# sczhou/CodeFormer

Hardware: AMD Instinct MI355X
Metric: aligned 512x512 faces/sec (whole node) at w=0.5 (higher is better)
Workload: dtype f32; 1 GPU; BASELINE config 2 (IEEE fp32 arithmetic): 16 faces/GPU, w=0.5, adain, seed-0 random-init weights; global_batch=16, parallelism=single GPU, precision=fp32

## Files before the change

### codeformer_amd/csrc/cf_gemm_split.hip

```cpp
#include <cstdlib>
#include <type_traits>

#include "cf_common.h"

namespace {

typedef _Float16 gs_f16x8 __attribute__((ext_vector_type(8)));

struct GsArgs {
  const float* a;
  const float* w;
  const float* bias;
  const float* res;
  float* out;
  int M, N, K;
  int epilogue;
  float acc_scale;
  float* ws;
  unsigned* counters;
  int nsplit;
  const float* a_alt;
  int n_alt;
};
__device__ __forceinline__ const float* gs_rows(const GsArgs& g, int n0) { return (g.a_alt && n0 >= g.n_alt) ? g.a_alt : g.a; }

constexpr int GS_GROUP = 4;

__global__ __launch_bounds__(256) void gemm_split_kernel(const GsArgs g) {
  __shared__ float s_flag;
  const int tid = threadIdx.x, lane = tid & 63, wave = tid >> 6;
  const int wm = wave >> 1, wn = wave & 1;
  const int half = lane >> 5, l31 = lane & 31;
  int bid = blockIdx.x;
  const int split = bid % g.nsplit;
  const int tile = bid / g.nsplit;
  const int ntn = g.N >> 6;
  const int nt = tile % ntn, mt = tile / ntn;
  const int m0 = mt * 64 + wm * 32, n0 = nt * 64 + wn * 32;
  const int V = g.K >> 7;
  const int nv = V / g.nsplit;
  const int c0 = split * nv;

  const float* const arow = gs_rows(g, n0) + (size_t)(m0 + l31) * g.K + half * 8 + (size_t)c0 * 128;
  const size_t kstride = (size_t)(g.N >> 5) * 512;
  const float* const wl = g.w + (size_t)(n0 >> 5) * 512 + lane * 4 + (size_t)c0 * 8 * kstride;

  f32x4 ra[2][GS_GROUP][2], rb[2][GS_GROUP][2];
  auto fetch = [&](int grp, auto buf) __attribute__((always_inline)) {
    constexpr int BUF = decltype(buf)::value;
#pragma unroll
    for (int s = 0; s < GS_GROUP; ++s) {
      const int ks = grp * GS_GROUP + s;
      ra[BUF][s][0] = *reinterpret_cast<const f32x4*>(arow + ks * 16);
      ra[BUF][s][1] = *reinterpret_cast<const f32x4*>(arow + ks * 16 + 4);
      rb[BUF][s][0] = *reinterpret_cast<const f32x4*>(wl + (size_t)ks * kstride);
      rb[BUF][s][1] = *reinterpret_cast<const f32x4*>(wl + (size_t)ks * kstride + 256);
    }
  };
  f32x16 acc, tot;
#pragma unroll
  for (int r = 0; r < 16; ++r) acc[r] = tot[r] = 0.f;
  auto compute = [&](auto buf) __attribute__((always_inline)) {
    constexpr int BUF = decltype(buf)::value;
#pragma unroll
    for (int s = 0; s < GS_GROUP; ++s) {
      f32x4 ah, al;
#pragma unroll
      for (int e = 0; e < 4; ++e) {
        const f32x4 v = ra[BUF][s][e >> 1];
        float hh, ll;
        cf_split_pair(v[(e & 1) * 2], v[(e & 1) * 2 + 1], hh, ll);
        ah[e] = hh;
        al[e] = ll;
      }
      acc = __builtin_amdgcn_mfma_f32_32x32x16_f16(__builtin_bit_cast(gs_f16x8, al), __builtin_bit_cast(gs_f16x8, rb[BUF][s][0]), acc, 0, 0, 0);
      acc = __builtin_amdgcn_mfma_f32_32x32x16_f16(__builtin_bit_cast(gs_f16x8, ah), __builtin_bit_cast(gs_f16x8, rb[BUF][s][1]), acc, 0, 0, 0);
      acc = __builtin_amdgcn_mfma_f32_32x32x16_f16(__builtin_bit_cast(gs_f16x8, ah), __builtin_bit_cast(gs_f16x8, rb[BUF][s][0]), acc, 0, 0, 0);
    }
  };

  using B0 = std::integral_constant<int, 0>;
  using B1 = std::integral_constant<int, 1>;
  const int ngroups = nv * 2;
  fetch(0, B0{});
  for (int c = 0; c < nv; ++c) {
    fetch(2 * c + 1, B1{});
    __builtin_amdgcn_sched_barrier(0);
    compute(B0{});
    if (2 * c + 2 < ngroups) fetch(2 * c + 2, B0{});
    __builtin_amdgcn_sched_barrier(0);
    compute(B1{});
    if (g.nsplit == 1) {
#pragma unroll
      for (int r = 0; r < 16; ++r) tot[r] += acc[r];
    } else {
      f32x4 v[4];
#pragma unroll
      for (int i = 0; i < 4; ++i) v[i] = f32x4{acc[4 * i], acc[4 * i + 1], acc[4 * i + 2], acc[4 * i + 3]};
      cf_splitk_park(v, g.ws, tile, c0 + c, V, 256);
    }
#pragma unroll
    for (int r = 0; r < 16; ++r) acc[r] = 0.f;
  }
  if (g.nsplit > 1) {
    f32x4 v[4];
    if (!cf_splitk_finish(v, g.ws, g.counters, tile, V, g.nsplit, 256, &s_flag)) return;
#pragma unroll
    for (int i = 0; i < 4; ++i)
#pragma unroll
      for (int e = 0; e < 4; ++e) tot[4 * i + e] = v[i][e];
  }

  const int n = n0 + l31;
  const float bias = g.bias ? g.bias[n] : 0.f;
#pragma unroll
  for (int r = 0; r < 16; ++r) {
    const size_t o = (size_t)(m0 + cf_acc_row(r, lane)) * g.N + n;
    float v = tot[r] * g.acc_scale + bias;
    if (g.epilogue == CF_EPI_GELU) v = 0.5f * v * (1.0f + erff(v * 0.70710678118654752440f));
    if (g.epilogue == CF_EPI_RESIDUAL) v += g.res[o];
    g.out[o] = v;
  }
}

template <int NI>
__global__ __launch_bounds__(256) void gemm_split_tile_kernel(const GsArgs g) {
  constexpr int BN = 64 * NI;
  __shared__ __attribute__((aligned(16))) float As[2][2][128][16];
  const int tid = threadIdx.x, lane = tid & 63, wave = __builtin_amdgcn_readfirstlane(tid >> 6);
  const int wm = wave >> 1, wn = wave & 1;
  const int half = lane >> 5, l31 = lane & 31;
  const int ntn = g.N / BN;
  const int nt = blockIdx.x % ntn, mt = blockIdx.x / ntn;
  const int m0 = mt * 128, n0 = nt * BN + wn * (32 * NI);
  const int nst = g.K >> 5;

  const float* const asrc = gs_rows(g, n0) + (size_t)(m0 + (tid >> 3)) * g.K + (tid & 7) * 4;
  f32x4 rg[4][4];
  auto load_stage = [&](int st, auto buf) __attribute__((always_inline)) {
    constexpr int BUF = decltype(buf)::value;
#pragma unroll
    for (int j = 0; j < 4; ++j) rg[BUF][j] = *reinterpret_cast<const f32x4*>(asrc + (size_t)(32 * j) * g.K + st * 32);
  };
  typedef float gs_f32x2 __attribute__((ext_vector_type(2)));
  auto store_stage = [&](int lbuf, auto buf) __attribute__((always_inline)) {
    constexpr int BUF = decltype(buf)::value;
    const int q = tid & 7, ks = q >> 2, hf = (q >> 1) & 1, sub = q & 1;
#pragma unroll
    for (int j = 0; j < 4; ++j) {
      const int row = (tid >> 3) + 32 * j;
      const int swz = (row >> 2) & 3;
      float h0, l0, h1, l1;
      cf_split_pair(rg[BUF][j][0], rg[BUF][j][1], h0, l0);
      cf_split_pair(rg[BUF][j][2], rg[BUF][j][3], h1, l1);
      float* base = &As[lbuf][ks][row][0];
      *reinterpret_cast<gs_f32x2*>(base + ((hf ^ swz) << 2) + sub * 2) = gs_f32x2{h0, h1};
      *reinterpret_cast<gs_f32x2*>(base + (((2 + hf) ^ swz) << 2) + sub * 2) = gs_f32x2{l0, l1};
    }
  };
  const size_t kstride = (size_t)(g.N >> 5) * 512;
  const float* const wl = g.w + (size_t)(n0 >> 5) * 512 + lane * 4;
  f32x4 rb[4][2][NI][2];
  auto load_B = [&](int st, auto buf) __attribute__((always_inline)) {
    constexpr int BUF = decltype(buf)::value;
#pragma unroll
    for (int s = 0; s < 2; ++s)
#pragma unroll
      for (int ni = 0; ni < NI; ++ni) {
        const float* p = wl + (size_t)(st * 2 + s) * kstride + ni * 512;
        rb[BUF][s][ni][0] = *reinterpret_cast<const f32x4*>(p);
        rb[BUF][s][ni][1] = *reinterpret_cast<const f32x4*>(p + 256);
      }
  };
  f32x16 acc[2][NI], tot[2][NI];
#pragma unroll
  for (int mi = 0; mi < 2; ++mi)
#pragma unroll
    for (int ni = 0; ni < NI; ++ni)
#pragma unroll
      for (int r = 0; r < 16; ++r) acc[mi][ni][r] = tot[mi][ni][r] = 0.f;
  auto compute = [&](int lbuf, auto buf) __attribute__((always_inline)) {
    constexpr int BUF = decltype(buf)::value;
#pragma unroll
    for (int s = 0; s < 2; ++s) {
      f32x4 ah[2], al[2];
#pragma unroll
      for (int mi = 0; mi < 2; ++mi) {
        const int row = wm * 64 + mi * 32 + l31;
        const int swz = (row >> 2) & 3;
        ah[mi] = *reinterpret_cast<const f32x4*>(&As[lbuf][s][row][(half ^ swz) << 2]);
        al[mi] = *reinterpret_cast<const f32x4*>(&As[lbuf][s][row][((2 + half) ^ swz) << 2]);
      }
#pragma unroll
      for (int mi = 0; mi < 2; ++mi)
#pragma unroll
        for (int ni = 0; ni < NI; ++ni) {
          acc[mi][ni] = __builtin_amdgcn_mfma_f32_32x32x16_f16(__builtin_bit_cast(gs_f16x8, al[mi]), __builtin_bit_cast(gs_f16x8, rb[BUF][s][ni][0]), acc[mi][ni], 0, 0, 0);
          acc[mi][ni] = __builtin_amdgcn_mfma_f32_32x32x16_f16(__builtin_bit_cast(gs_f16x8, ah[mi]), __builtin_bit_cast(gs_f16x8, rb[BUF][s][ni][1]), acc[mi][ni], 0, 0, 0);
          acc[mi][ni] = __builtin_amdgcn_mfma_f32_32x32x16_f16(__builtin_bit_cast(gs_f16x8, ah[mi]), __builtin_bit_cast(gs_f16x8, rb[BUF][s][ni][0]), acc[mi][ni], 0, 0, 0);
        }
    }
  };
  using R0 = std::integral_constant<int, 0>;
  using R1 = std::integral_constant<int, 1>;
  using R2 = std::integral_constant<int, 2>;
  using R3 = std::integral_constant<int, 3>;
  auto stage = [&](int st, auto cur, auto nxt, auto far, auto do_load, auto do_store) __attribute__((always_inline)) {
    if constexpr (decltype(do_load)::value) {
      load_stage(st + 3, far);
      load_B(st + 3, far);
    }
    __builtin_amdgcn_sched_barrier(0);
    compute(st & 1, cur);
    if ((st & 3) == 3) {
#pragma unroll
      for (int mi = 0; mi < 2; ++mi)
#pragma unroll
        for (int ni = 0; ni < NI; ++ni)
#pragma unroll
          for (int r = 0; r < 16; ++r) {
            tot[mi][ni][r] += acc[mi][ni][r];
            acc[mi][ni][r] = 0.f;
          }
    }
    if constexpr (decltype(do_store)::value) store_stage((st + 1) & 1, nxt);
    __syncthreads();
  };
  constexpr std::true_type Y{};
  constexpr std::false_type NO{};
  load_stage(0, R0{});
  load_B(0, R0{});
  load_stage(1, R1{});
  load_B(1, R1{});
  load_stage(2, R2{});
  load_B(2, R2{});
  store_stage(0, R0{});
  __syncthreads();
  int st = 0;
  for (; st + 4 < nst; st += 4) {
    stage(st, R0{}, R1{}, R3{}, Y, Y);
    stage(st + 1, R1{}, R2{}, R0{}, Y, Y);
    stage(st + 2, R2{}, R3{}, R1{}, Y, Y);
    stage(st + 3, R3{}, R0{}, R2{}, Y, Y);
  }
  stage(st, R0{}, R1{}, R3{}, Y, Y);
  stage(st + 1, R1{}, R2{}, R0{}, NO, Y);
  stage(st + 2, R2{}, R3{}, R1{}, NO, Y);
  stage(st + 3, R3{}, R0{}, R2{}, NO, NO);

#pragma unroll
  for (int ni = 0; ni < NI; ++ni) {
    const int n = n0 + ni * 32 + l31;
    const float bias = g.bias ? g.bias[n] : 0.f;
#pragma unroll
    for (int mi = 0; mi < 2; ++mi)
#pragma unroll
      for (int r = 0; r < 16; ++r) {
        const size_t o = (size_t)(m0 + wm * 64 + mi * 32 + cf_acc_row(r, lane)) * g.N + n;
        float v = tot[mi][ni][r] * g.acc_scale + bias;
        if (g.epilogue == CF_EPI_GELU) v = 0.5f * v * (1.0f + erff(v * 0.70710678118654752440f));
        if (g.epilogue == CF_EPI_RESIDUAL) v += g.res[o];
        g.out[o] = v;
      }
  }
}

constexpr int GS_CHUNK_MAXV = 8;
template <int MI, int NI>
__global__ __launch_bounds__(256, MI * NI == 1 ? 1 : 2) void gemm_split_chunk_kernel(const GsArgs g) {
  extern __shared__ __attribute__((aligned(16))) float gs_part[];
  constexpr int HS = MI * NI == 1 ? 8 : 4;
  const int tid = threadIdx.x, lane = tid & 63, wave = __builtin_amdgcn_readfirstlane(tid >> 6);
  const int half = lane >> 5, l31 = lane & 31;
  const int ntn = g.N / (32 * NI);
  const int nt = blockIdx.x % ntn, mt = blockIdx.x / ntn;
  const int m0 = mt * (32 * MI), n0 = nt * (32 * NI);
  const int V = g.K >> 7;
  const float* const arow = gs_rows(g, n0) + (size_t)(m0 + l31) * g.K + half * 8;
  const size_t kstride = (size_t)(g.N >> 5) * 512;
  const float* const wl = g.w + (size_t)(n0 >> 5) * 512 + lane * 4;
  for (int c = wave; c < V; c += 4) {
    f32x16 acc[MI][NI];
#pragma unroll
    for (int mi = 0; mi < MI; ++mi)
#pragma unroll
      for (int ni = 0; ni < NI; ++ni)
#pragma unroll
        for (int r = 0; r < 16; ++r) acc[mi][ni][r] = 0.f;
#pragma unroll
    for (int h = 0; h < 8 / HS; ++h) {
      f32x4 ra[HS][MI][2], rb[HS][NI][2];
#pragma unroll
      for (int s = 0; s < HS; ++s) {
        const int ks = c * 8 + h * HS + s;
#pragma unroll
        for (int mi = 0; mi < MI; ++mi) {
          ra[s][mi][0] = *reinterpret_cast<const f32x4*>(arow + (size_t)(32 * mi) * g.K + ks * 16);
          ra[s][mi][1] = *reinterpret_cast<const f32x4*>(arow + (size_t)(32 * mi) * g.K + ks * 16 + 4);
        }
#pragma unroll
        for (int ni = 0; ni < NI; ++ni) {
          rb[s][ni][0] = *reinterpret_cast<const f32x4*>(wl + (size_t)ks * kstride + ni * 512);
          rb[s][ni][1] = *reinterpret_cast<const f32x4*>(wl + (size_t)ks * kstride + ni * 512 + 256);
        }
      }
      __builtin_amdgcn_sched_barrier(0);
#pragma unroll
      for (int s = 0; s < HS; ++s) {
        f32x4 ah[MI], al[MI];
#pragma unroll
        for (int mi = 0; mi < MI; ++mi)
#pragma unroll
          for (int e = 0; e < 4; ++e) {
            const f32x4 v = ra[s][mi][e >> 1];
            float hh, ll;
            cf_split_pair(v[(e & 1) * 2], v[(e & 1) * 2 + 1], hh, ll);
            ah[mi][e] = hh;
            al[mi][e] = ll;
          }
#pragma unroll
        for (int mi = 0; mi < MI; ++mi)
#pragma unroll
          for (int ni = 0; ni < NI; ++ni) {
            acc[mi][ni] = __builtin_amdgcn_mfma_f32_32x32x16_f16(__builtin_bit_cast(gs_f16x8, al[mi]), __builtin_bit_cast(gs_f16x8, rb[s][ni][0]), acc[mi][ni], 0, 0, 0);
            acc[mi][ni] = __builtin_amdgcn_mfma_f32_32x32x16_f16(__builtin_bit_cast(gs_f16x8, ah[mi]), __builtin_bit_cast(gs_f16x8, rb[s][ni][1]), acc[mi][ni], 0, 0, 0);
            acc[mi][ni] = __builtin_amdgcn_mfma_f32_32x32x16_f16(__builtin_bit_cast(gs_f16x8, ah[mi]), __builtin_bit_cast(gs_f16x8, rb[s][ni][0]), acc[mi][ni], 0, 0, 0);
          }
      }
    }
#pragma unroll
    for (int mi = 0; mi < MI; ++mi)
#pragma unroll
      for (int ni = 0; ni < NI; ++ni)
#pragma unroll
        for (int r = 0; r < 16; ++r) gs_part[(((c * MI + mi) * NI + ni) * 16 + r) * 64 + lane] = acc[mi][ni][r];
  }
  __syncthreads();
#pragma unroll
  for (int ni = 0; ni < NI; ++ni) {
    const int n = n0 + ni * 32 + l31;
    const float bias = g.bias ? g.bias[n] : 0.f;
#pragma unroll
    for (int mi = 0; mi < MI; ++mi)
#pragma unroll
      for (int j = 0; j < 4; ++j) {
        const int r = wave + 4 * j;
        float tot = 0.f;
        for (int c = 0; c < V; ++c) tot += gs_part[(((c * MI + mi) * NI + ni) * 16 + r) * 64 + lane];
        const size_t o = (size_t)(m0 + mi * 32 + cf_acc_row(r, lane)) * g.N + n;
        float v = tot * g.acc_scale + bias;
        if (g.epilogue == CF_EPI_GELU) v = 0.5f * v * (1.0f + erff(v * 0.70710678118654752440f));
        if (g.epilogue == CF_EPI_RESIDUAL) v += g.res[o];
        g.out[o] = v;
      }
  }
}

__global__ __launch_bounds__(256) void gemm_f32_tile_kernel(const GsArgs g) {
  __shared__ __attribute__((aligned(16))) float As[2][2][128][16];
  const int tid = threadIdx.x, lane = tid & 63, wave = __builtin_amdgcn_readfirstlane(tid >> 6);
  const int wm = wave >> 1, wn = wave & 1;
  const int half = lane >> 5, l31 = lane & 31;
  const int ntn = g.N / 64;
  const int nt = blockIdx.x % ntn, mt = blockIdx.x / ntn;
  const int m0 = mt * 128, n0 = nt * 64 + wn * 32;
  const int nst = g.K >> 5;

  const float* const asrc = gs_rows(g, n0) + (size_t)(m0 + (tid >> 3)) * g.K + (tid & 7) * 4;
  f32x4 rg[4][4];
  auto load_stage = [&](int st, auto buf) __attribute__((always_inline)) {
    constexpr int BUF = decltype(buf)::value;
#pragma unroll
    for (int j = 0; j < 4; ++j) rg[BUF][j] = *reinterpret_cast<const f32x4*>(asrc + (size_t)(32 * j) * g.K + st * 32);
  };
  auto store_stage = [&](int lbuf, auto buf) __attribute__((always_inline)) {
    constexpr int BUF = decltype(buf)::value;
    const int q = tid & 7, ks = q >> 2, ch = q & 3;
#pragma unroll
    for (int j = 0; j < 4; ++j) {
      const int row = (tid >> 3) + 32 * j;
      *reinterpret_cast<f32x4*>(&As[lbuf][ks][row][(ch ^ ((row >> 2) & 3)) << 2]) = rg[BUF][j];
    }
  };
  const float* const wl = g.w + (size_t)(n0 + l31) * 16 + half * 4;
  const size_t kstride = (size_t)g.N * 16;
  f32x4 rb[4][2][2];
  auto load_B = [&](int st, auto buf) __attribute__((always_inline)) {
    constexpr int BUF = decltype(buf)::value;
#pragma unroll
    for (int s = 0; s < 2; ++s) {
      const float* p = wl + (size_t)(st * 2 + s) * kstride;
      rb[BUF][s][0] = *reinterpret_cast<const f32x4*>(p);
      rb[BUF][s][1] = *reinterpret_cast<const f32x4*>(p + 8);
    }
  };
  f32x16 acc[2], tot[2];
#pragma unroll
  for (int mi = 0; mi < 2; ++mi)
#pragma unroll
    for (int r = 0; r < 16; ++r) acc[mi][r] = tot[mi][r] = 0.f;
  auto compute = [&](int lbuf, auto buf) __attribute__((always_inline)) {
    constexpr int BUF = decltype(buf)::value;
#pragma unroll
    for (int s = 0; s < 2; ++s) {
      f32x4 a0[2], a1[2];
#pragma unroll
      for (int mi = 0; mi < 2; ++mi) {
        const int row = wm * 64 + mi * 32 + l31;
        const int swz = (row >> 2) & 3;
        a0[mi] = *reinterpret_cast<const f32x4*>(&As[lbuf][s][row][(half ^ swz) << 2]);
        a1[mi] = *reinterpret_cast<const f32x4*>(&As[lbuf][s][row][((2 + half) ^ swz) << 2]);
      }
#pragma unroll
      for (int j = 0; j < 4; ++j)
#pragma unroll
        for (int mi = 0; mi < 2; ++mi) acc[mi] = __builtin_amdgcn_mfma_f32_32x32x2f32(a0[mi][j], rb[BUF][s][0][j], acc[mi], 0, 0, 0);
#pragma unroll
      for (int j = 0; j < 4; ++j)
#pragma unroll
        for (int mi = 0; mi < 2; ++mi) acc[mi] = __builtin_amdgcn_mfma_f32_32x32x2f32(a1[mi][j], rb[BUF][s][1][j], acc[mi], 0, 0, 0);
    }
  };
  using R0 = std::integral_constant<int, 0>;
  using R1 = std::integral_constant<int, 1>;
  using R2 = std::integral_constant<int, 2>;
  using R3 = std::integral_constant<int, 3>;
  auto stage = [&](int st, auto cur, auto nxt, auto far, auto do_load, auto do_store) __attribute__((always_inline)) {
    if constexpr (decltype(do_load)::value) {
      load_stage(st + 3, far);
      load_B(st + 3, far);
    }
    __builtin_amdgcn_sched_barrier(0);
    compute(st & 1, cur);
    if ((st & 3) == 3) {
#pragma unroll
      for (int mi = 0; mi < 2; ++mi) {
        tot[mi] += acc[mi];
#pragma unroll
        for (int r = 0; r < 16; ++r) acc[mi][r] = 0.f;
      }
    }
    if constexpr (decltype(do_store)::value) store_stage((st + 1) & 1, nxt);
    __syncthreads();
  };
  constexpr std::true_type Y{};
  constexpr std::false_type NO{};
  load_stage(0, R0{});
  load_B(0, R0{});
  load_stage(1, R1{});
  load_B(1, R1{});
  load_stage(2, R2{});
  load_B(2, R2{});
  store_stage(0, R0{});
  __syncthreads();
  int st = 0;
  for (; st + 4 < nst; st += 4) {
    stage(st, R0{}, R1{}, R3{}, Y, Y);
    stage(st + 1, R1{}, R2{}, R0{}, Y, Y);
    stage(st + 2, R2{}, R3{}, R1{}, Y, Y);
    stage(st + 3, R3{}, R0{}, R2{}, Y, Y);
  }
  stage(st, R0{}, R1{}, R3{}, Y, Y);
  stage(st + 1, R1{}, R2{}, R0{}, NO, Y);
  stage(st + 2, R2{}, R3{}, R1{}, NO, Y);
  stage(st + 3, R3{}, R0{}, R2{}, NO, NO);

  const int n = n0 + l31;
  const float bias = g.bias ? g.bias[n] : 0.f;
#pragma unroll
  for (int mi = 0; mi < 2; ++mi)
#pragma unroll
    for (int r = 0; r < 16; ++r) {
      const size_t o = (size_t)(m0 + wm * 64 + mi * 32 + cf_acc_row(r, lane)) * g.N + n;
      float v = tot[mi][r] + bias;
      if (g.epilogue == CF_EPI_GELU) v = 0.5f * v * (1.0f + erff(v * 0.70710678118654752440f));
      if (g.epilogue == CF_EPI_RESIDUAL) v += g.res[o];
      g.out[o] = v;
    }
}

__global__ void pack_linear_f16x2_kernel(const float* __restrict__ w, int N, int K, float scale, unsigned* __restrict__ packed, long total) {
  const long i = (long)blockIdx.x * blockDim.x + threadIdx.x;
  if (i >= total) return;
  const int e = (int)(i & 3), ln = (int)((i >> 2) & 63), part = (int)((i >> 8) & 1);
  long r = i >> 9;
  const int ntiles = N / 32;
  const int n = (int)(r % ntiles) * 32 + (ln & 31);
  const int ks = (int)(r / ntiles);
  unsigned out = 0;
#pragma unroll
  for (int h = 0; h < 2; ++h) {
    const int k = ks * 16 + (ln >> 5) * 8 + e * 2 + h;
    const float v = w[(long)n * K + k] * scale;
    const _Float16 hi = (_Float16)v;
    const _Float16 hv = part ? (_Float16)(v - (float)hi) : hi;
    out |= (unsigned)__builtin_bit_cast(unsigned short, hv) << (16 * h);
  }
  packed[i] = out;
}

}

extern "C" int cf_pack_linear_weight_f16x2(const float* w, int n, int k, float scale, void* packed, cf_stream_t stream) {
  CF_REQUIRE(w && packed, "cf_pack_linear_weight_f16x2: null pointer");
  CF_REQUIRE(n > 0 && k > 0 && n % 64 == 0 && k % 128 == 0, "cf_pack_linear_weight_f16x2: N %d must be a multiple of 64, K %d of 128", n, k);
  int ex = 0;
  CF_REQUIRE(scale > 0.f && frexpf(scale, &ex) == 0.5f, "cf_pack_linear_weight_f16x2: scale %g is not a power of two", (double)scale);
  const long total = (long)n * k;
  hipLaunchKernelGGL(pack_linear_f16x2_kernel, dim3((unsigned)((total + 255) / 256)), dim3(256), 0, (hipStream_t)stream, w, n, k, scale,
                     reinterpret_cast<unsigned*>(packed), total);
  CF_CHECK_LAUNCH("cf_pack_linear_weight_f16x2");
  return CF_OK;
}

int cf_gemm_split_geometry(const cf_conv_desc* d, int* tiles, long* bytes_per_part) {
  const long m = (long)d->batch * d->hout * d->wout;
  const int mq = d->split_k == CF_SPLITK_IN_WORKGROUP ? 32 : 64;
  CF_REQUIRE(d->taps == 1 && m % mq == 0 && d->cout % 64 == 0 && d->cout_pad == d->cout && (d->c0 + d->c1) % 128 == 0,
             "cf_conv2d(1x1, f16x2): M %ld must be a multiple of %d, N %d of 64, K %d of 128", m, mq, d->cout, d->c0 + d->c1);
  *tiles = (int)(m / 64) * (d->cout / 64);
  const int V = (d->c0 + d->c1) / 128;
  *bytes_per_part = 64L * 64 * 4 * V / (d->split_k > 0 ? d->split_k : 1);
  return CF_OK;
}

int cf_gemm_split_launch(const cf_conv_desc* d, hipStream_t stream) {
  int tiles = 0;
  long per = 0;
  const int rc = cf_gemm_split_geometry(d, &tiles, &per);
  if (rc != CF_OK) return rc;
  CF_REQUIRE(d->stride == 1 && !d->in_nchw && !d->out_nchw && d->c1 == 0 && d->prologue == CF_PRO_NONE && !d->stats_out &&
                 (d->ld_in0 == 0 || d->ld_in0 == d->c0) && (d->ld_out == 0 || d->ld_out == d->cout),
             "cf_conv2d(1x1, f16x2): dense single-input token GEMMs without prologue / statistics only");
  CF_REQUIRE(d->epilogue == CF_EPI_NONE || d->epilogue == CF_EPI_GELU || d->epilogue == CF_EPI_RESIDUAL,
             "cf_conv2d(1x1, f16x2): epilogues are none / GELU / residual");
  CF_REQUIRE(d->acc_scale > 0.f, "cf_conv2d(1x1, f16x2): acc_scale must be the inverse of the pack-time weight scale (got %g)", (double)d->acc_scale);
  CF_REQUIRE(!d->in0_alt || (d->alt_cout0 > 0 && d->alt_cout0 < d->cout && d->alt_cout0 % 128 == 0),
             "cf_conv2d(1x1, f16x2): in0_alt needs 0 < alt_cout0 < cout, a multiple of 128 (got %d of %d)", d->alt_cout0, d->cout);
  const int V = d->c0 / 128;
  if (d->split_k == CF_SPLITK_IN_WORKGROUP) {
    const long m = (long)d->batch * d->hout * d->wout;
    CF_REQUIRE(V >= 1 && V <= GS_CHUNK_MAXV && m % 32 == 0,
               "cf_conv2d(1x1, f16x2, in-workgroup split): K %d must be a multiple of 128 up to %d, M a multiple of 32 (N %% 64 == 0: the packing)", d->c0, GS_CHUNK_MAXV * 128);
    GsArgs g;
    g.a_alt = d->in0_alt;
    g.n_alt = d->alt_cout0;
    g.a = d->in0;
    g.w = d->weight;
    g.bias = d->bias;
    g.res = d->res;
    g.out = d->out;
    g.M = (int)m;
    g.N = d->cout;
    g.K = d->c0;
    g.epilogue = d->epilogue;
    g.acc_scale = d->acc_scale;
    g.ws = nullptr;
    g.counters = nullptr;
    g.nsplit = 1;
    CF_LDS_ATTR((gemm_split_chunk_kernel<1, 1>), GS_CHUNK_MAXV * 4096);
    hipLaunchKernelGGL((gemm_split_chunk_kernel<1, 1>), dim3((unsigned)((g.M / 32) * (g.N / 32))), dim3(256), (size_t)V * 4096, stream, g);
    CF_CHECK_LAUNCH("cf_conv2d(1x1, f16x2, in-workgroup split)");
    return CF_OK;
  }
  const int nsplit = d->split_k >= 1 ? d->split_k : 1;
  CF_REQUIRE(V % nsplit == 0, "cf_conv2d(1x1, f16x2): split_k %d must divide K/128 = %d", nsplit, V);
  CF_REQUIRE(nsplit == 1 || (d->workspace && d->counters), "cf_conv2d(1x1, f16x2): split_k > 1 needs workspace and counters");
  GsArgs g;
  g.a_alt = d->in0_alt;
  g.n_alt = d->alt_cout0;
  g.a = d->in0;
  g.w = d->weight;
  g.bias = d->bias;
  g.res = d->res;
  g.out = d->out;
  g.M = (int)((long)d->batch * d->hout * d->wout);
  g.N = d->cout;
  g.K = d->c0;
  g.epilogue = d->epilogue;
  g.acc_scale = d->acc_scale;
  g.ws = d->workspace;
  g.counters = d->counters;
  g.nsplit = nsplit;
  if (nsplit == 1 && g.M % 128 == 0 && g.K % 64 == 0) {
    hipLaunchKernelGGL(gemm_split_tile_kernel<1>, dim3((unsigned)((g.M / 128) * (g.N / 64))), dim3(256), 0, stream, g);
    CF_CHECK_LAUNCH("cf_conv2d(1x1, f16x2, token tiles)");
    return CF_OK;
  }
  hipLaunchKernelGGL(gemm_split_kernel, dim3((unsigned)(tiles * nsplit)), dim3(256), 0, stream, g);
  CF_CHECK_LAUNCH("cf_conv2d(1x1, f16x2)");
  return CF_OK;
}

int cf_gemm_f32_tile_try(const cf_conv_desc* d, hipStream_t stream) {
  const long m = (long)d->batch * d->hout * d->wout;
  const int k = d->c0;
  if (d->taps != 1 || d->bf16_mfma != CF_OPERAND_F32 || d->split_k != 1 || d->c1 != 0 || d->stride != 1 || d->in_nchw || d->out_nchw ||
      d->prologue != CF_PRO_NONE || d->stats_out || d->stats_cpg || m % 128 || k % 128 || d->cout % 64 || d->cout_pad != d->cout ||
      (d->ld_in0 != 0 && d->ld_in0 != d->c0) || (d->ld_out != 0 && d->ld_out != d->cout) || d->pad_mode != CF_PAD_ZERO ||
      !(d->epilogue == CF_EPI_NONE || d->epilogue == CF_EPI_GELU || d->epilogue == CF_EPI_RESIDUAL))
    return 1;
  if (k == 512 && d->cout == 512) return 1;
  GsArgs g;
  g.a_alt = nullptr;
  g.n_alt = 0;
  g.a = d->in0;
  g.w = d->weight;
  g.bias = d->bias;
  g.res = d->res;
  g.out = d->out;
  g.M = (int)m;
  g.N = d->cout;
  g.K = k;
  g.epilogue = d->epilogue;
  g.acc_scale = 1.f;
  g.ws = nullptr;
  g.counters = nullptr;
  g.nsplit = 1;
  hipLaunchKernelGGL(gemm_f32_tile_kernel, dim3((unsigned)((g.M / 128) * (g.N / 64))), dim3(256), 0, stream, g);
  CF_CHECK_LAUNCH("cf_conv2d(1x1, fp32 token tiles)");
  return CF_OK;
}
```

### codeformer_amd/lib.py

```python
import ctypes
import os

import torch

_PKG = os.path.dirname(os.path.abspath(__file__))
LIB_PATH = os.environ.get('CF_LIB_PATH') or os.path.join(_PKG, 'libcodeformer_hip.so')

c_float_p = ctypes.c_void_p

ABI_VERSION = 22
PRO_NONE, PRO_AFFINE, PRO_AFFINE_SWISH, PRO_LEAKY = 0, 1, 2, 3
EPI_NONE, EPI_RESIDUAL, EPI_SFT, EPI_GELU, EPI_LEAKY, EPI_AXPY, EPI_AXPY2 = 0, 1, 2, 3, 4, 5, 6
PAD_ZERO, PAD_REFLECT, PAD_EDGE = 0, 1, 2


class ConvDesc(ctypes.Structure):
    _fields_ = [
        ('in0', ctypes.c_void_p), ('in1', ctypes.c_void_p),
        ('c0', ctypes.c_int32), ('c1', ctypes.c_int32),
        ('batch', ctypes.c_int32), ('hin', ctypes.c_int32), ('win', ctypes.c_int32),
        ('hout', ctypes.c_int32), ('wout', ctypes.c_int32),
        ('cout', ctypes.c_int32), ('cout_pad', ctypes.c_int32),
        ('taps', ctypes.c_int32), ('stride', ctypes.c_int32), ('upsample', ctypes.c_int32),
        ('in_nchw', ctypes.c_int32), ('out_nchw', ctypes.c_int32),
        ('prologue', ctypes.c_int32), ('epilogue', ctypes.c_int32),
        ('pro_scale', ctypes.c_void_p), ('pro_shift', ctypes.c_void_p),
        ('weight', ctypes.c_void_p), ('bias', ctypes.c_void_p),
        ('res', ctypes.c_void_p), ('sft_scale', ctypes.c_void_p),
        ('sft_w', ctypes.c_float),
        ('out', ctypes.c_void_p),
        ('stats_out', ctypes.c_void_p), ('stats_cpg', ctypes.c_int32), ('bf16_mfma', ctypes.c_int32),
        ('ld_in0', ctypes.c_int32), ('ld_in1', ctypes.c_int32), ('ld_out', ctypes.c_int32),
        ('pad_mode', ctypes.c_int32), ('pad_lo', ctypes.c_int32), ('winograd', ctypes.c_int32),
        ('acc_scale', ctypes.c_float),
        ('split_k', ctypes.c_int32), ('workspace', ctypes.c_void_p), ('counters', ctypes.c_void_p),
        ('act_scale', ctypes.c_void_p),
        ('io_bf16', ctypes.c_int32),
        ('in0_alt', ctypes.c_void_p), ('alt_cout0', ctypes.c_int32),
    ]


_I, _P, _F, _L = ctypes.c_int, ctypes.c_void_p, ctypes.c_float, ctypes.c_int64
SIGNATURES = {
    'cf_version': (_I, []),
    'cf_last_error': (ctypes.c_char_p, []),
    'cf_build_id': (ctypes.c_char_p, []),
    'cf_device_cu_count': (_I, []),
    'cf_device_init': (_I, []),
    'cf_conv2d': (_I, [ctypes.POINTER(ConvDesc), _P]),
    'cf_conv2d_stats_parts': (_I, [ctypes.POINTER(ConvDesc)]),
    'cf_conv2d_workspace_bytes': (_L, [ctypes.POINTER(ConvDesc)]),
    'cf_conv2d_tiles': (_I, [ctypes.POINTER(ConvDesc)]),
    'cf_pack_conv_weight': (_I, [_P, _I, _I, _I, _I, _I, _P, _P]),
    'cf_packed_weight_elems': (_L, [_I, _I, _I]),
    'cf_pack_conv_weight_bf16': (_I, [_P, _I, _I, _I, _I, _I, _P, _P]),
    'cf_pack_conv_weight_f16': (_I, [_P, _I, _I, _I, _I, _I, _P, _P]),
    'cf_pack_conv_weight_up2x': (_I, [_P, _I, _I, _I, _I, _P, _P]),
    'cf_pack_conv_weight_winograd': (_I, [_P, _I, _I, _I, _I, _P, _P]),
    'cf_pack_conv_weight_winograd_f16x2': (_I, [_P, _I, _I, _I, _I, _F, _P, _P]),
    'cf_pack_conv_weight_winograd_bf16': (_I, [_P, _I, _I, _I, _I, _F, _P, _P]),
    'cf_pack_conv_weight_winograd43_f16x2': (_I, [_P, _I, _I, _I, _I, _F, _P, _P]),
    'cf_pack_conv_weight_winograd43': (_I, [_P, _I, _I, _I, _I, _P, _P]),
    'cf_pack_linear_weight_f16x2': (_I, [_P, _I, _I, _F, _P, _P]),
    'cf_pack_conv_weight_up2x_bf16': (_I, [_P, _I, _I, _I, _I, _P, _P]),
    'cf_pack_conv_weight_up2x_f16': (_I, [_P, _I, _I, _I, _I, _P, _P]),
    'cf_pack_conv_weight_f16x2': (_I, [_P, _I, _I, _I, _I, _I, _F, _P, _P]),
    'cf_groupnorm_stats': (_I, [_P, _I, _I, _I, _I, _P, _I, _P]),
    'cf_act_scale_from_stats': (_I, [_P, _I, _I, _F, _P, _P, _P]),
    'cf_act_scale_from_tensor': (_I, [_P, _I, _L, _F, _P, _P, _P]),
    'cf_act_scale_fused': (_I, [_P, _I, _P, _I, _P, _L, _I, _F, _P, _P, _P]),
    'cf_groupnorm_finalize': (_I, [_P, _I, _I, _I, _I, _I, _L, _P, _P, _F, _P, _P, _I, _P]),
    'cf_groupnorm_finalize2': (_I, [_P, _I, _I, _I, _I, _P, _I, _I, _I, _I, _I, _L, _P, _P, _F, _P, _P, _I, _F, _P, _P, _P]),
    'cf_layernorm': (_I, [_P, _I, _I, _P, _P, _F, _P, _I, _P, _P, _P]),
    'cf_attention': (_I, [_P, _I, _P, _I, _P, _I, _P, _I, _I, _I, _I, _I, _F, _P]),
    'cf_argmax_rows': (_I, [_P, _I, _I, _P, _P]),
    'cf_codebook_gather_adain': (_I, [_P, _P, _I, _P, _I, _I, _I, _I, _F, _P, _P]),
    'cf_row_sqnorm': (_I, [_P, _I, _I, _P, _P]),
    'cf_vq_argmin': (_I, [_P, _P, _P, _I, _I, _P, _P, _P]),
    'cf_nchw_to_nhwc': (_I, [_P, _I, _I, _I, _P, _P]),
    'cf_pixel_unshuffle_nhwc': (_I, [_P, _I, _I, _I, _I, _I, _I, _P, _P]),
    'cf_nhwc_to_nchw': (_I, [_P, _I, _I, _I, _P, _P]),
    'cf_img_u8_to_tensor': (_I, [_P, _I, _I, _I, _P, _P]),
    'cf_tensor_to_img_u8': (_I, [_P, _I, _I, _I, _P, _P]),
    'cf_mask_composite': (_I, [_P, _P, _I, _I, _I, _P, _P]),
    'cf_f32_to_bf16': (_I, [_P, _L, _P, _P]),
    'cf_fused_bias_act': (_I, [_P, _P, _L, _I, _I, _F, _F, _P, _P]),
    'cf_fused_bias_act_ex': (_I, [_P, _P, _P, _L, _I, _I, _I, _I, _F, _F, _I, _P, _P]),
    'cf_upfirdn2d': (_I, [_P, _I, _I, _I, _P, _I, _I, _I, _I, _I, _I, _I, _I, _I, _I, _P, _P]),
    'cf_warp_affine_u8': (_I, [_P, _L, _I, _I, _P, _I, _P, _I, _I, _I, _I, _I, _I, _I, _I, _I, _P]),
    'cf_warp_affine_f32': (_I, [_P, _I, _I, ctypes.POINTER(ctypes.c_double), _P, _I, _I, _I, _I, _P]),
    'cf_erode_f32': (_I, [_P, _P, _P, _I, _I, _I, _P]),
    'cf_gaussian_blur_f32': (_I, [_P, _P, _P, _I, _I, _I, _I, _I, _I, _P, _I, _P]),
    'cf_sum_f32': (_I, [_P, _L, _P, _P]),
    'cf_paste_blend': (_I, [_P, _I, _I, _P, _I, _I, ctypes.POINTER(ctypes.c_double), _P, _P, _P, _I, _I, _I, _I, _P]),
    'cf_resize_linear_u8': (_I, [_P, _I, _I, _P, _I, _I, _P]),
    'cf_resize_area_u8': (_I, [_P, _I, _I, _P, _I, _I, _P]),
    'cf_f32_to_u8_trunc': (_I, [_P, _L, _P, _P]),
    'cf_label_lut_f32': (_I, [_P, _L, ctypes.POINTER(ctypes.c_float), _I, _P, _P]),
    'cf_scale_clear_border_f32': (_I, [_P, _I, _I, _I, _I, _F, _P]),
    'cf_box_overlay_u8': (_I, [_P, _I, _I, _P, _I, _I, _I, _P, _P]),
    'cf_resize_linear_f32': (_I, [_P, _I, _I, _I, _P, _I, _I, _P]),
    'cf_esrgan_tile_gather_u8': (_I, [_P, _I, _I, _I, _I, _I, _I, _I, _I, _I, _P, _P]),
    'cf_esrgan_tile_scatter_u8': (_I, [_P, _I, _I, _I, _I, _I, _I, _I, _P, _I, _I, _I, _I, _P]),
}

_lib = None
_cuda = None
_devices = set()


class NativeLibraryError(RuntimeError):
    pass


def load():
    global _cuda
    lib = _lib if _lib is not None else _open()
    if _cuda is None:
        _cuda = torch.cuda.is_available()
    if _cuda:
        dev = torch.cuda.current_device()
        if dev not in _devices:
            _init_device(lib, dev)
    return lib


def _init_device(lib, dev):
    if torch.cuda.is_current_stream_capturing():
        raise NativeLibraryError(f'cf_device_init has not run on cuda:{dev} yet and the current stream is capturing: call '
                                 'codeformer_amd.lib.ensure_device(device) (or run one forward) before the capture')
    if lib.cf_device_init() != 0:
        raise NativeLibraryError(f'cf_device_init failed on cuda:{dev} ({torch.cuda.get_device_name(dev)}): '
                                 f'{lib.cf_last_error().decode("utf-8", "replace")}')
    _devices.add(dev)


def ensure_device(device):
    global _cuda
    lib = _lib if _lib is not None else _open()
    if _cuda is None:
        _cuda = torch.cuda.is_available()
    if not _cuda:
        return lib
    d = torch.device(device) if not isinstance(device, int) else torch.device('cuda', device)
    idx = torch.cuda.current_device() if d.index is None else d.index
    if idx not in _devices:
        with torch.cuda.device(idx):
            _init_device(lib, idx)
    return lib


def _open():
    global _lib
    if not os.path.exists(LIB_PATH):
        raise NativeLibraryError(
            f'{LIB_PATH} not found: build it with `python -m codeformer_amd.build` (hipcc --offload-arch=gfx950). '
            'codeformer_amd has no non-HIP execution path for GPU tensors.')
    try:
        lib = ctypes.CDLL(LIB_PATH)
    except OSError as e:
        raise NativeLibraryError(f'cannot load {LIB_PATH}: {e}') from e
    for name, (res, args) in SIGNATURES.items():
        fn = getattr(lib, name)
        fn.restype = res
        fn.argtypes = args
    if lib.cf_version() != ABI_VERSION:
        raise NativeLibraryError(f'ABI version mismatch: library {lib.cf_version()}, binding {ABI_VERSION}')
    _lib = lib
    return lib


def is_available():
    return os.path.exists(LIB_PATH)


def last_error():
    lib = _lib if _lib is not None else _open()
    return lib.cf_last_error().decode('utf-8', 'replace')


def check(status, what):
    if status != 0:
        raise RuntimeError(f'{what} failed ({status}): {last_error()}')


def stream_ptr():
    return torch.cuda.current_stream().cuda_stream


def ptr(t, strided=False, dtype=torch.float32):
    if t is None:
        return None
    if not t.is_cuda:
        raise ValueError('codeformer_amd ops need CUDA (ROCm) tensors')
    if dtype is not None and t.dtype != dtype:
        raise TypeError(f'codeformer_amd op expected a {dtype} tensor, got {t.dtype}')
    if not strided and not t.is_contiguous():
        raise ValueError('codeformer_amd ops need contiguous tensors')
    return t.data_ptr()
```

### include/codeformer_hip.h

```cpp
#ifndef CODEFORMER_HIP_H
#define CODEFORMER_HIP_H

#include <stdint.h>

#ifdef __cplusplus
extern "C" {
#endif

#define CF_ABI_VERSION 22
#define CF_SPLITK_IN_WORKGROUP (-1)

typedef void* cf_stream_t;

enum cf_status {
  CF_OK = 0,
  CF_ERR_ARG = -1,
  CF_ERR_LAUNCH = -2,
};

int cf_version(void);
const char* cf_build_id(void);
const char* cf_last_error(void);
int cf_device_cu_count(void);
int cf_device_init(void);

enum cf_prologue {
  CF_PRO_NONE = 0,
  CF_PRO_AFFINE = 1,
  CF_PRO_AFFINE_SWISH = 2,
  CF_PRO_LEAKY = 3,
};
enum cf_epilogue {
  CF_EPI_NONE = 0,
  CF_EPI_RESIDUAL = 1,
  CF_EPI_SFT = 2,
  CF_EPI_GELU = 3,
  CF_EPI_LEAKY = 4,
  CF_EPI_AXPY = 5,
  CF_EPI_AXPY2 = 6,
};

enum cf_operand {
  CF_OPERAND_F32 = 0,
  CF_OPERAND_BF16 = 1,
  CF_OPERAND_F16 = 2,
  CF_OPERAND_F16X2 = 3,
};

enum cf_pad {
  CF_PAD_ZERO = 0,
  CF_PAD_REFLECT = 1,
  CF_PAD_EDGE = 2,
};

typedef struct cf_conv_desc {
  const float* in0;
  const float* in1;
  int32_t c0, c1;
  int32_t batch, hin, win;
  int32_t hout, wout;
  int32_t cout;
  int32_t cout_pad;
  int32_t taps;
  int32_t stride;
  int32_t upsample;
  int32_t in_nchw;
  int32_t out_nchw;
  int32_t prologue;
  int32_t epilogue;
  const float* pro_scale;
  const float* pro_shift;
  const float* weight;
  const float* bias;
  const float* res;
  const float* sft_scale;
  float sft_w;
  float* out;
  double* stats_out;
  int32_t stats_cpg;
  int32_t bf16_mfma;
  int32_t ld_in0, ld_in1, ld_out;
  int32_t pad_mode;
  int32_t pad_lo;
  int32_t winograd;
  float acc_scale;
  int32_t split_k;
  float* workspace;
  uint32_t* counters;
  const float* act_scale;
  int32_t io_bf16;
  const float* in0_alt;
  int32_t alt_cout0;
} cf_conv_desc;

int cf_conv2d(const cf_conv_desc* d, cf_stream_t stream);
int cf_conv2d_stats_parts(const cf_conv_desc* d);
int64_t cf_conv2d_workspace_bytes(const cf_conv_desc* d);
int cf_conv2d_tiles(const cf_conv_desc* d);

int cf_pack_conv_weight(const float* w, int cout, int cin, int taps, int cout_pad, int cin_pad,
                        float* packed, cf_stream_t stream);
int64_t cf_packed_weight_elems(int cin_pad, int taps, int cout_pad);
int cf_pack_conv_weight_winograd(const float* w, int cout, int cin, int cout_pad, int cin_pad, float* packed, cf_stream_t stream);
int cf_pack_conv_weight_winograd_f16x2(const float* w, int cout, int cin, int cout_pad, int cin_pad, float scale, void* packed,
                                       cf_stream_t stream);
int cf_pack_conv_weight_winograd43_f16x2(const float* w, int cout, int cin, int cout_pad, int cin_pad, float scale, void* packed,
                                         cf_stream_t stream);
int cf_pack_conv_weight_winograd43(const float* w, int cout, int cin, int cout_pad, int cin_pad, void* packed, cf_stream_t stream);
int cf_pack_conv_weight_winograd_bf16(const float* w, int cout, int cin, int cout_pad, int cin_pad, float scale, void* packed,
                                      cf_stream_t stream);
int cf_pack_linear_weight_f16x2(const float* w, int n, int k, float scale, void* packed, cf_stream_t stream);
int cf_pack_conv_weight_bf16(const float* w, int cout, int cin, int taps, int cout_pad, int cin_pad, void* packed,
                             cf_stream_t stream);
int cf_pack_conv_weight_up2x(const float* w, int cout, int cin, int cout_pad, int cin_pad, float* packed, cf_stream_t stream);
int cf_pack_conv_weight_up2x_bf16(const float* w, int cout, int cin, int cout_pad, int cin_pad, void* packed,
                                  cf_stream_t stream);
int cf_pack_conv_weight_f16(const float* w, int cout, int cin, int taps, int cout_pad, int cin_pad, void* packed,
                            cf_stream_t stream);
int cf_pack_conv_weight_up2x_f16(const float* w, int cout, int cin, int cout_pad, int cin_pad, void* packed,
                                 cf_stream_t stream);
int cf_pack_conv_weight_f16x2(const float* w, int cout, int cin, int up2x, int cout_pad, int cin_pad, float scale, void* packed,
                              cf_stream_t stream);

int cf_groupnorm_stats(const float* x, int batch, int hw, int c, int cpg, double* partial, int parts,
                       cf_stream_t stream);
int cf_act_scale_from_stats(const double* partial, int batch, int nper, float growth, float* scratch, float* act, cf_stream_t stream);
int cf_act_scale_from_tensor(const float* x, int batch, int64_t n_per_image, float growth, float* scratch, float* act, cf_stream_t stream);
int cf_act_scale_fused(const double* partial_a, int nper_a, const double* partial_b, int nper_b, const float* x, int64_t n_per_image, int batch,
                       float growth, uint32_t* cells, float* act, cf_stream_t stream);
int cf_groupnorm_finalize(const double* partial, int batch, int parts, int c, int cpg, int gmerge, int64_t count,
                          const float* gamma, const float* beta, float eps, float* scale, float* shift, int ld,
                          cf_stream_t stream);
int cf_groupnorm_finalize2(const double* partial_a, int parts_a, int c_a, int cpg_a, int gmerge_a, const double* partial_b, int parts_b, int c_b,
                           int cpg_b, int gmerge_b, int batch, int64_t count, const float* gamma, const float* beta, float eps, float* scale,
                           float* shift, int ld, float act_growth, uint32_t* cells, float* act, cf_stream_t stream);

int cf_layernorm(const float* x, int rows, int c, const float* gamma, const float* beta, float eps,
                 const float* pos, int npos, float* y, float* ypos, cf_stream_t stream);

int cf_attention(const float* q, int ldq, const float* k, int ldk, const float* v, int ldv, float* out, int ldo,
                 int batch, int heads, int head_dim, int nkeys, float scale, cf_stream_t stream);

int cf_argmax_rows(const float* logits, int rows, int n, int64_t* idx, cf_stream_t stream);

int cf_codebook_gather_adain(const int64_t* idx, const float* codebook, int codebook_size, const float* lq,
                             int batch, int ntok, int dim, int adain, float eps, float* out, cf_stream_t stream);

int cf_row_sqnorm(const float* x, int rows, int dim, float* out, cf_stream_t stream);
int cf_vq_argmin(const float* scores, const float* zz, const float* ee, int rows, int ncodes, int64_t* idx,
                 float* dist_min, cf_stream_t stream);

int cf_nchw_to_nhwc(const float* x, int batch, int c, int hw, float* y, cf_stream_t stream);
int cf_nhwc_to_nchw(const float* x, int batch, int c, int hw, float* y, cf_stream_t stream);

int cf_pixel_unshuffle_nhwc(const float* x, int batch, int c, int h, int w, int s, int c_pad, float* out, cf_stream_t stream);

int cf_img_u8_to_tensor(const uint8_t* img, int batch, int h, int w, float* out, cf_stream_t stream);
int cf_tensor_to_img_u8(const float* t, int batch, int h, int w, uint8_t* img, cf_stream_t stream);
int cf_mask_composite(const float* x, const float* y, int batch, int h, int w, float* out, cf_stream_t stream);
int cf_f32_to_bf16(const float* x, int64_t numel, void* out, cf_stream_t stream);

int cf_fused_bias_act(const float* x, const float* bias, int64_t numel, int c, int hw, float slope, float scale,
                      float* y, cf_stream_t stream);
int cf_fused_bias_act_ex(const void* x, const void* bias, const void* ref, int64_t numel, int c, int hw, int act, int grad, float alpha,
                         float scale, int dtype, void* y, cf_stream_t stream);
int cf_upfirdn2d(const float* x, int nplanes, int in_h, int in_w, const float* kernel, int kh, int kw, int up_x,
                 int up_y, int down_x, int down_y, int pad_x0, int pad_x1, int pad_y0, int pad_y1, float* y,
                 cf_stream_t stream);

int cf_warp_affine_u8(const uint8_t* src, int64_t src_stride, int sh, int sw, const double* inv_dev, int n, uint8_t* dst, int dh, int dw,
                      int rx, int ry, int rw, int rh, int b0, int b1, int b2, cf_stream_t stream);
int cf_warp_affine_f32(const float* src, int sh, int sw, const double* inv_host, float* dst_region, int rx, int ry, int rw, int rh,
                       cf_stream_t stream);
int cf_erode_f32(const float* in_region, float* tmp_region, float* out_region, int rh, int rw, int k, cf_stream_t stream);
int cf_gaussian_blur_f32(const float* in_region, float* tmp_region, float* out_region, int rh, int rw, int rx, int ry, int ch, int cw,
                         const float* taps_dev, int ksize, cf_stream_t stream);
int cf_sum_f32(const float* x, int64_t n, double* partials64, cf_stream_t stream);
int cf_paste_blend(float* canvas, int ch, int cw, const uint8_t* face, int fh, int fw, const double* inv_host, const float* ero_region,
                   const float* soft_region, const float* parse_region, int rx, int ry, int rw, int rh, cf_stream_t stream);
int cf_resize_linear_u8(const uint8_t* src, int sh, int sw, float* dst, int dh, int dw, cf_stream_t stream);
int cf_resize_area_u8(const uint8_t* src, int sh, int sw, uint8_t* dst, int dh, int dw, cf_stream_t stream);
int cf_f32_to_u8_trunc(const float* src, int64_t n, uint8_t* dst, cf_stream_t stream);
int cf_label_lut_f32(const int64_t* labels, int64_t n, const float* lut_host, int nlut, float* out, cf_stream_t stream);
int cf_scale_clear_border_f32(float* x, int batch, int h, int w, int border, float scale, cf_stream_t stream);
int cf_box_overlay_u8(const float* canvas, int ch, int cw, const double* faces_dev, int nfaces, int fh, int fw, uint8_t* out,
                      cf_stream_t stream);
int cf_resize_linear_f32(const float* src, int batch, int sh, int sw, float* dst, int dh, int dw, cf_stream_t stream);
int cf_esrgan_tile_gather_u8(const uint8_t* faces, int n, int h, int w, int pre_pad, int mod, int py0, int px0, int th, int tw, float* out,
                             cf_stream_t stream);
int cf_esrgan_tile_scatter_u8(const float* up, int n, int uh, int uw, int oy, int ox, int ch, int cw, uint8_t* out, int oh, int ow, int dy,
                              int dx, cf_stream_t stream);

#ifdef __cplusplus
}
#endif
#endif
```

Measured before the change: 344.0 faces/s.

## Add intra-block split-K pair GEMM kernel and XCD-major block remap for fp32 GEMMs

```diff
diff --git a/codeformer_amd/csrc/cf_gemm_split.hip b/codeformer_amd/csrc/cf_gemm_split.hip
--- a/codeformer_amd/csrc/cf_gemm_split.hip
+++ b/codeformer_amd/csrc/cf_gemm_split.hip
@@ -24,6 +24,8 @@
 };
 __device__ __forceinline__ const float* gs_rows(const GsArgs& g, int n0) { return (g.a_alt && n0 >= g.n_alt) ? g.a_alt : g.a; }
 
+__device__ __forceinline__ int gs_xcd_major(int b, int nb) { return (nb & 7) ? b : (b & 7) * (nb >> 3) + (b >> 3); }
+
 constexpr int GS_GROUP = 4;
 
 __global__ __launch_bounds__(256) void gemm_split_kernel(const GsArgs g) {
@@ -362,7 +364,8 @@
   const int wm = wave >> 1, wn = wave & 1;
   const int half = lane >> 5, l31 = lane & 31;
   const int ntn = g.N / 64;
-  const int nt = blockIdx.x % ntn, mt = blockIdx.x / ntn;
+  const int bid = gs_xcd_major(blockIdx.x, gridDim.x);
+  const int nt = bid % ntn, mt = bid / ntn;
   const int m0 = mt * 128, n0 = nt * 64 + wn * 32;
   const int nst = g.K >> 5;
 
@@ -477,6 +480,152 @@
       if (g.epilogue == CF_EPI_RESIDUAL) v += g.res[o];
       g.out[o] = v;
     }
+}
+
+constexpr int GP_STAGE_FLOATS = 2 * 128 * 16;
+constexpr int GP_LDS_BYTES = (2 * 2 * GP_STAGE_FLOATS + 2 * 4 * 16 * 64) * 4;
+__global__ __launch_bounds__(512) void gemm_f32_pair_kernel(const GsArgs g) {
+  extern __shared__ __attribute__((aligned(16))) float gp_lds[];
+  const int grp = __builtin_amdgcn_readfirstlane(threadIdx.x >> 8);
+  const int tid = threadIdx.x & 255, lane = tid & 63, wave = __builtin_amdgcn_readfirstlane(tid >> 6);
+  const int wm = wave >> 1, wn = wave & 1;
+  const int half = lane >> 5, l31 = lane & 31;
+  const int ntn = g.N / 64;
+  const int bid = gs_xcd_major(blockIdx.x, gridDim.x);
+  const int nt = bid % ntn, mt = bid / ntn;
+  const int m0 = mt * 128, n0 = nt * 64 + wn * 32;
+  const int nls = g.K >> 6;
+  float* const As = gp_lds + grp * (2 * GP_STAGE_FLOATS);
+  f32x4* const park_mine = reinterpret_cast<f32x4*>(gp_lds + 4 * GP_STAGE_FLOATS) + ((grp * 4 + wave) * 4) * 64 + lane;
+  const f32x4* const park_theirs = reinterpret_cast<const f32x4*>(gp_lds + 4 * GP_STAGE_FLOATS) + (((grp ^ 1) * 4 + wave) * 4) * 64 + lane;
+  auto kst = [&](int ls) __attribute__((always_inline)) { return ((ls >> 2) * 2 + grp) * 4 + (ls & 3); };
+
+  const float* const asrc = g.a + (size_t)(m0 + (tid >> 3)) * g.K + (tid & 7) * 4;
+  f32x4 rg[4][4];
+  auto load_stage = [&](int ls, auto buf) __attribute__((always_inline)) {
+    constexpr int BUF = decltype(buf)::value;
+    const int st = kst(ls);
+#pragma unroll
+    for (int j = 0; j < 4; ++j) rg[BUF][j] = *reinterpret_cast<const f32x4*>(asrc + (size_t)(32 * j) * g.K + st * 32);
+  };
+  auto store_stage = [&](int lbuf, auto buf) __attribute__((always_inline)) {
+    constexpr int BUF = decltype(buf)::value;
+    const int q = tid & 7, ks = q >> 2, ch = q & 3;
+#pragma unroll
+    for (int j = 0; j < 4; ++j) {
+      const int row = (tid >> 3) + 32 * j;
+      *reinterpret_cast<f32x4*>(As + lbuf * GP_STAGE_FLOATS + (ks * 128 + row) * 16 + ((ch ^ ((row >> 2) & 3)) << 2)) = rg[BUF][j];
+    }
+  };
+  const float* const wl = g.w + (size_t)(n0 + l31) * 16 + half * 4;
+  const size_t kstride = (size_t)g.N * 16;
+  f32x4 rb[4][2][2];
+  auto load_B = [&](int ls, auto buf) __attribute__((always_inline)) {
+    constexpr int BUF = decltype(buf)::value;
+    const int st = kst(ls);
+#pragma unroll
+    for (int s = 0; s < 2; ++s) {
+      const float* p = wl + (size_t)(st * 2 + s) * kstride;
+      rb[BUF][s][0] = *reinterpret_cast<const f32x4*>(p);
+      rb[BUF][s][1] = *reinterpret_cast<const f32x4*>(p + 8);
+    }
+  };
+  f32x16 acc[2], tot;
+#pragma unroll
+  for (int r = 0; r < 16; ++r) acc[0][r] = acc[1][r] = tot[r] = 0.f;
+  auto compute = [&](int lbuf, auto buf) __attribute__((always_inline)) {
+    constexpr int BUF = decltype(buf)::value;
+#pragma unroll
+    for (int s = 0; s < 2; ++s) {
+      f32x4 a0[2], a1[2];
+#pragma unroll
+      for (int mi = 0; mi < 2; ++mi) {
+        const int row = wm * 64 + mi * 32 + l31;
+        const int swz = (row >> 2) & 3;
+        const float* base = As + lbuf * GP_STAGE_FLOATS + (s * 128 + row) * 16;
+        a0[mi] = *reinterpret_cast<const f32x4*>(base + ((half ^ swz) << 2));
+        a1[mi] = *reinterpret_cast<const f32x4*>(base + (((2 + half) ^ swz) << 2));
+      }
+#pragma unroll
+      for (int j = 0; j < 4; ++j)
+#pragma unroll
+        for (int mi = 0; mi < 2; ++mi) acc[mi] = __builtin_amdgcn_mfma_f32_32x32x2f32(a0[mi][j], rb[BUF][s][0][j], acc[mi], 0, 0, 0);
+#pragma unroll
+      for (int j = 0; j < 4; ++j)
+#pragma unroll
+        for (int mi = 0; mi < 2; ++mi) acc[mi] = __builtin_amdgcn_mfma_f32_32x32x2f32(a1[mi][j], rb[BUF][s][1][j], acc[mi], 0, 0, 0);
+    }
+  };
+  using R0 = std::integral_constant<int, 0>;
+  using R1 = std::integral_constant<int, 1>;
+  using R2 = std::integral_constant<int, 2>;
+  using R3 = std::integral_constant<int, 3>;
+  auto stage = [&](int ls, auto cur, auto nxt, auto far, auto do_load, auto do_store) __attribute__((always_inline)) {
+    if constexpr (decltype(do_load)::value) {
+      load_stage(ls + 3, far);
+      load_B(ls + 3, far);
+    }
+    __builtin_amdgcn_sched_barrier(0);
+    compute(ls & 1, cur);
+    const bool chunk_done = (ls & 3) == 3;
+    if (chunk_done) {
+      const f32x16& give = grp == 0 ? acc[1] : acc[0];
+#pragma unroll
+      for (int i = 0; i < 4; ++i) park_mine[i * 64] = f32x4{give[4 * i], give[4 * i + 1], give[4 * i + 2], give[4 * i + 3]};
+    }
+    if constexpr (decltype(do_store)::value) store_stage((ls + 1) & 1, nxt);
+    __syncthreads();
+    if (chunk_done) {
+      f32x16 got;
+#pragma unroll
+      for (int i = 0; i < 4; ++i) {
+        const f32x4 v = park_theirs[i * 64];
+#pragma unroll
+        for (int e = 0; e < 4; ++e) got[4 * i + e] = v[e];
+      }
+      if (grp == 0) {
+        tot += acc[0];
+        tot += got;
+      } else {
+        tot += got;
+        tot += acc[1];
+      }
+#pragma unroll
+      for (int r = 0; r < 16; ++r) acc[0][r] = acc[1][r] = 0.f;
+    }
+  };
+  constexpr std::true_type Y{};
+  constexpr std::false_type NO{};
+  load_stage(0, R0{});
+  load_B(0, R0{});
+  load_stage(1, R1{});
+  load_B(1, R1{});
+  load_stage(2, R2{});
+  load_B(2, R2{});
+  store_stage(0, R0{});
+  __syncthreads();
+  int ls = 0;
+  for (; ls + 4 < nls; ls += 4) {
+    stage(ls, R0{}, R1{}, R3{}, Y, Y);
+    stage(ls + 1, R1{}, R2{}, R0{}, Y, Y);
+    stage(ls + 2, R2{}, R3{}, R1{}, Y, Y);
+    stage(ls + 3, R3{}, R0{}, R2{}, Y, Y);
+  }
+  stage(ls, R0{}, R1{}, R3{}, Y, Y);
+  stage(ls + 1, R1{}, R2{}, R0{}, NO, Y);
+  stage(ls + 2, R2{}, R3{}, R1{}, NO, Y);
+  stage(ls + 3, R3{}, R0{}, R2{}, NO, NO);
+
+  const int n = n0 + l31;
+  const float bias = g.bias ? g.bias[n] : 0.f;
+#pragma unroll
+  for (int r = 0; r < 16; ++r) {
+    const size_t o = (size_t)(m0 + wm * 64 + grp * 32 + cf_acc_row(r, lane)) * g.N + n;
+    float v = tot[r] + bias;
+    if (g.epilogue == CF_EPI_GELU) v = 0.5f * v * (1.0f + erff(v * 0.70710678118654752440f));
+    if (g.epilogue == CF_EPI_RESIDUAL) v += g.res[o];
+    g.out[o] = v;
+  }
 }
 
 __global__ void pack_linear_f16x2_kernel(const float* __restrict__ w, int N, int K, float scale, unsigned* __restrict__ packed, long total) {
@@ -592,15 +741,23 @@
   return CF_OK;
 }
 
-int cf_gemm_f32_tile_try(const cf_conv_desc* d, hipStream_t stream) {
+extern "C" int cf_gemm_f32_form(const cf_conv_desc* d) {
+  if (!d) return CF_GEMM_F32_FORM_SPLITK;
   const long m = (long)d->batch * d->hout * d->wout;
   const int k = d->c0;
   if (d->taps != 1 || d->bf16_mfma != CF_OPERAND_F32 || d->split_k != 1 || d->c1 != 0 || d->stride != 1 || d->in_nchw || d->out_nchw ||
       d->prologue != CF_PRO_NONE || d->stats_out || d->stats_cpg || m % 128 || k % 128 || d->cout % 64 || d->cout_pad != d->cout ||
       (d->ld_in0 != 0 && d->ld_in0 != d->c0) || (d->ld_out != 0 && d->ld_out != d->cout) || d->pad_mode != CF_PAD_ZERO ||
-      !(d->epilogue == CF_EPI_NONE || d->epilogue == CF_EPI_GELU || d->epilogue == CF_EPI_RESIDUAL))
-    return 1;
-  if (k == 512 && d->cout == 512) return 1;
+      !(d->epilogue == CF_EPI_NONE || d->epilogue == CF_EPI_GELU || d->epilogue == CF_EPI_RESIDUAL) || d->io_bf16)
+    return CF_GEMM_F32_FORM_SPLITK;
+  if (k == 512 && d->cout == 512 && m < 4096) return CF_GEMM_F32_FORM_SPLITK;
+  if (k % 256 == 0 && (m / 128) * (d->cout / 64) <= 256) return CF_GEMM_F32_FORM_PAIR;
+  return CF_GEMM_F32_FORM_TILE;
+}
+
+int cf_gemm_f32_tile_try(const cf_conv_desc* d, hipStream_t stream) {
+  const int form = cf_gemm_f32_form(d);
+  if (form == CF_GEMM_F32_FORM_SPLITK) return 1;
   GsArgs g;
   g.a_alt = nullptr;
   g.n_alt = 0;
@@ -609,15 +766,21 @@
   g.bias = d->bias;
   g.res = d->res;
   g.out = d->out;
-  g.M = (int)m;
+  g.M = (int)((long)d->batch * d->hout * d->wout);
   g.N = d->cout;
-  g.K = k;
+  g.K = d->c0;
   g.epilogue = d->epilogue;
   g.acc_scale = 1.f;
   g.ws = nullptr;
   g.counters = nullptr;
   g.nsplit = 1;
-  hipLaunchKernelGGL(gemm_f32_tile_kernel, dim3((unsigned)((g.M / 128) * (g.N / 64))), dim3(256), 0, stream, g);
+  const dim3 grid((unsigned)((g.M / 128) * (g.N / 64)));
+  if (form == CF_GEMM_F32_FORM_PAIR) {
+    CF_LDS_ATTR(gemm_f32_pair_kernel, GP_LDS_BYTES);
+    hipLaunchKernelGGL(gemm_f32_pair_kernel, grid, dim3(512), GP_LDS_BYTES, stream, g);
+  } else {
+    hipLaunchKernelGGL(gemm_f32_tile_kernel, grid, dim3(256), 0, stream, g);
+  }
   CF_CHECK_LAUNCH("cf_conv2d(1x1, fp32 token tiles)");
   return CF_OK;
 }
diff --git a/codeformer_amd/lib.py b/codeformer_amd/lib.py
--- a/codeformer_amd/lib.py
+++ b/codeformer_amd/lib.py
@@ -51,6 +51,7 @@
     'cf_conv2d_stats_parts': (_I, [ctypes.POINTER(ConvDesc)]),
     'cf_conv2d_workspace_bytes': (_L, [ctypes.POINTER(ConvDesc)]),
     'cf_conv2d_tiles': (_I, [ctypes.POINTER(ConvDesc)]),
+    'cf_gemm_f32_form': (_I, [ctypes.POINTER(ConvDesc)]),
     'cf_pack_conv_weight': (_I, [_P, _I, _I, _I, _I, _I, _P, _P]),
     'cf_packed_weight_elems': (_L, [_I, _I, _I]),
     'cf_pack_conv_weight_bf16': (_I, [_P, _I, _I, _I, _I, _I, _P, _P]),
diff --git a/include/codeformer_hip.h b/include/codeformer_hip.h
--- a/include/codeformer_hip.h
+++ b/include/codeformer_hip.h
@@ -97,6 +97,10 @@
 int cf_conv2d_stats_parts(const cf_conv_desc* d);
 int64_t cf_conv2d_workspace_bytes(const cf_conv_desc* d);
 int cf_conv2d_tiles(const cf_conv_desc* d);
+#define CF_GEMM_F32_FORM_SPLITK 0
+#define CF_GEMM_F32_FORM_TILE 1
+#define CF_GEMM_F32_FORM_PAIR 2
+int cf_gemm_f32_form(const cf_conv_desc* d);
 
 int cf_pack_conv_weight(const float* w, int cout, int cin, int taps, int cout_pad, int cin_pad,
                         float* packed, cf_stream_t stream);
```

New measurement: 345.0 faces/s (median of 6 runs). Within noise of the previous version (+0.3%).
